# anacarsi/ss25_Hierarchical_Multiscale_Image_Classification

Measured on AMD Instinct MI355X. Metric: 224x224 patches/sec (ResNet18 fwd), higher is better.
Workload: dtype bf16; 1 GPU; resnet18_fwd_872k_patches_bf16; input=uint8 HWC patches resident in HBM, outputs=features[B,512] + logits[B,2] + labels, weights=seeded random init, parallelism=single GPU

## Files before the change

### ss25_hierarchical_multiscale_image_classification_amd/csrc/halo16.h

```cpp
#pragma once
#include "conv_device.h"

namespace hipac {

template <typename T> struct Elem16;
template <> struct Elem16<__bf16> {
  static __device__ __forceinline__ f32x4 mfma(bf16x8 a, bf16x8 b, f32x4 c) {
    return __builtin_amdgcn_mfma_f32_16x16x32_bf16(a, b, c, 0, 0, 0);
  }
};
template <> struct Elem16<_Float16> {
  static __device__ __forceinline__ f32x4 mfma(f16x8 a, f16x8 b, f32x4 c) {
    return __builtin_amdgcn_mfma_f32_16x16x32_f16(a, b, c, 0, 0, 0);
  }
};

template <typename T> struct Asm16;
template <> struct Asm16<__bf16> {
  static __device__ __forceinline__ void mfma(f32x4& c, const bf16x8& a, const bf16x8& b) {
    asm volatile("v_mfma_f32_16x16x32_bf16 %0, %1, %2, %0" : "+v"(c) : "v"(a), "v"(b));
  }
};
template <> struct Asm16<_Float16> {
  static __device__ __forceinline__ void mfma(f32x4& c, const f16x8& a, const f16x8& b) {
    asm volatile("v_mfma_f32_16x16x32_f16 %0, %1, %2, %0" : "+v"(c) : "v"(a), "v"(b));
  }
};
template <int OFF, typename F>
__device__ __forceinline__ void lds_read16(F& f, unsigned addr) {
  static_assert(OFF >= 0 && OFF < 65536, "ds offset field");
  asm volatile("ds_read_b128 %0, %1 offset:%2" : "=v"(f) : "v"(addr), "n"(OFF));
}
#if defined(__HIP_DEVICE_COMPILE__)
__device__ __forceinline__ void permlane16_swap(unsigned& a, unsigned& b) {
  const auto r = __builtin_amdgcn_permlane16_swap(a, b, false, false);
  a = r[0];
  b = r[1];
}
#else
__device__ inline void permlane16_swap(unsigned&, unsigned&) {}
#endif
template <int N>
__device__ __forceinline__ void wait_lgkmcnt() {
  static_assert(N >= 0 && N < 16, "lgkmcnt range");
  asm volatile("s_waitcnt lgkmcnt(%0)" ::"n"(N));
}

template <int STRIDE> __host__ __device__ constexpr int b16_tap(int k) { return STRIDE == 1 ? k : (int)((0x471538620ull >> (4 * k)) & 15); }
template <int STRIDE> __host__ __device__ constexpr int b16_kh(int k) { return b16_tap<STRIDE>(k) / 3; }
template <int STRIDE> __host__ __device__ constexpr int b16_kw(int k) { return b16_tap<STRIDE>(k) % 3; }
__host__ __device__ constexpr int perm16(int n) { return n < 4 ? 2 * n : (n < 12 ? 2 * n - 7 : 2 * n - 16); }
__host__ __device__ constexpr int perm16_inv(int j) { return (j & 1) ? (j + 7) / 2 : (j < 8 ? j / 2 : j / 2 + 8); }

#ifndef HIPAC_H16_EPI_PRIO
#define HIPAC_H16_EPI_PRIO 0
#endif
#ifndef HIPAC_H16_STAGE16
#define HIPAC_H16_STAGE16 0
#endif
#ifndef HIPAC_H16_ABL
#define HIPAC_H16_ABL 0
#endif
#ifndef HIPAC_H16_AHEAD
#define HIPAC_H16_AHEAD 3
#endif

constexpr int kPoolSlots = 7;

#if defined(__HIP_DEVICE_COMPILE__)
template <int CTRL>
__device__ __forceinline__ float dpp_add(float v) {
  return v + __builtin_bit_cast(float, __builtin_amdgcn_update_dpp(0, __builtin_bit_cast(int, v), CTRL, 0xf, 0xf, false));
}
__device__ __forceinline__ float row16_sum(float v) {
  v = dpp_add<0x128>(v);
  v = dpp_add<0x124>(v);
  v = dpp_add<0x122>(v);
  return dpp_add<0x121>(v);
}
#else
__device__ inline float row16_sum(float v) { return v; }
#endif

template <typename T, int CIN, int COUT, int H, int W, int BM, int BN, int NSW, bool RELU, bool RESID, bool OUTF32, int PCIN = 0,
          bool POOL = false, bool S2 = false>
__global__ __launch_bounds__(256, 2) void conv3x3_halo16_kernel(const T* __restrict__ in, const T* __restrict__ wgt,
                                                                const float* __restrict__ bias, const T* __restrict__ resid,
                                                                void* __restrict__ outp, int M, int n_img, int n_mtiles,
                                                                const char* __restrict__ zero_page,
                                                                const T* __restrict__ wgt_p = nullptr) {
  using E = Elem<T>;
  using frag = typename E::frag;
  constexpr int CC = CIN / 64;
  constexpr int KTOT = 9 * CIN;
  constexpr int WM = 2, WN = 2;
  constexpr int WPX = BM / WM;
  constexpr int MT = WPX / 16;
  constexpr int WTN = BN / WN, NT = WTN / 16;
  constexpr int A_PIECES = halo_band_pieces(W, BM);
  constexpr int A_BYTES = A_PIECES * 1024;
  constexpr int W_BYTES = BN * 128;
  constexpr int WPW = BN / 8 / 4;
  constexpr int NTILES_N = COUT / BN;
  constexpr int PCC = PCIN / 64;
  constexpr int NSTEP = 9 * CC + PCC;
  static_assert(sizeof(T) == 2, "16-bit operands");
  static_assert(!S2 || (PCIN == 0 && !RESID && !POOL && !OUTF32), "stride-2 form: plain entry conv");
  static_assert(!POOL || (OUTF32 && RELU && (BM + H * W - 1) / (H * W) + 1 <= kPoolSlots && H * W > 16),
                "pooled epilogue: the fp32 form of the direct epilogue, maps of more than 16 pixels");
  static_assert(PCIN % 64 == 0 && (PCIN == 0 || !RESID), "folded projection replaces the residual input");
  static_assert((BM == 128 || BM == 256) && WTN % 16 == 0 && COUT % BN == 0 && CIN % 64 == 0 && MT <= 8, "tile shape");
  static_assert((BN / 8) % 4 == 0, "W piece split");
  static_assert(NSW == 2 || NSW == 3, "weight ring depth");
  constexpr int SROWW = WTN * 4 + 16;
  constexpr int STG_BYTES = 4 * 32 * SROWW;
  constexpr int S_BYTES = NSW * W_BYTES > STG_BYTES ? NSW * W_BYTES : STG_BYTES;
  static_assert(A_BYTES + S_BYTES <= 80 * 1024, "LDS: two workgroups per CU");
  static_assert(BM + 2 * W + 4 <= A_PIECES * 8, "band slots");

  extern __shared__ __attribute__((aligned(1024))) unsigned char ring[];
  unsigned char* const Abuf = ring;
  unsigned char* const Wbuf = ring + A_BYTES;

  const int tid = threadIdx.x;
  const int lane = tid & 63;
  const int wave = __builtin_amdgcn_readfirstlane(tid >> 6);
  const int wm = wave % WM, wn = wave / WM;
  const int n16 = lane & 15, g = lane >> 4;
  const int pn = n16 < 4 ? 2 * n16 : (n16 < 12 ? 2 * n16 - 7 : 2 * n16 - 16);

  using gptr_t = const __attribute__((address_space(1))) void*;
  using lptr_t = __attribute__((address_space(3))) void*;
  const char* in_b = reinterpret_cast<const char*>(in);
  const char* w_b = reinterpret_cast<const char*>(wgt);
  const int prow = lane >> 3, dchunk = lane & 7;

  const rsrc_t a_rsrc = make_rsrc(in_b, S2 ? n_img * (4 * H * W * CIN * 2) : M * CIN * 2);
  const int a_lane = (prow * CIN + (dchunk ^ ((4 * wave + (prow >> 1)) & 7)) * 8) * 2;
  constexpr int NPB = S2 ? (A_PIECES + 3) / 4 : 1;
  int b_pix[NPB];
  auto plane_offsets = [&](int m0_) {
    if constexpr (S2) {
#pragma unroll
      for (int k = 0; k < NPB; ++k) {
        const int q = 8 * (wave + 4 * k) + prow;
        const int u = m0_ - W - 3 + q;
        const int b = u / (H * W), rem = u - b * (H * W), r = rem / W, c = rem - r * W;
        b_pix[k] = (q >= 2 && u >= 0 && u < M) ? (b * (2 * H) + 2 * r) * (2 * W) + 2 * c : -1;
      }
    }
  };
  auto issue_plane_band = [&](int k, int cc) {
    if constexpr (S2) {
      const int py = k < 4 ? 1 : (k < 6 ? 0 : (k < 8 ? 1 : 0)), px = k < 6 ? 1 : 0;
      const int pofs = (py * 2 * W + px) * CIN * 2 + cc * 128 + (dchunk ^ ((4 * wave + (prow >> 1)) & 7)) * 16;
#pragma unroll
      for (int kk = 0; kk < NPB; ++kk) {
        const int p = wave + 4 * kk;
        if (p < A_PIECES) buffer_load_lds16(a_rsrc, Abuf + p * 1024, b_pix[kk] < 0 ? (int)0x80000000 : b_pix[kk] * (CIN * 2) + pofs, 0);
      }
    }
  };
  auto issue_band_of = [&](int m0_, int cc) {
    const int mlast_ = (m0_ + BM <= M ? m0_ + BM : M) - 1;
    const int npieces_ = (mlast_ - m0_ + 1 + 2 * W + 2 + 2 + 7) >> 3;
    const int base = ((m0_ - W - 3) * CIN + cc * 64) * 2;
    for (int p = wave; p < npieces_; p += 4) {
      int off = a_lane + base + p * (8 * CIN * 2);
      if (p == 0 && prow < 2) off = (int)0x80000000;
      buffer_load_lds16(a_rsrc, Abuf + p * 1024, off, 0);
    }
  };

  constexpr int N_EPI_STORES = MT * (OUTF32 ? NT : NT / 2);
  bool prev_full = false;
  for (int vb = blockIdx.x, first_tile = 1;; vb += gridDim.x, first_tile = 0) {
  const int xcd = vb & 7, slot = vb >> 3;
  const int mt_q = (n_mtiles + 7) >> 3;
  const int mt = (slot / NTILES_N) < mt_q ? xcd * mt_q + slot / NTILES_N : n_mtiles;
  const int nt = slot % NTILES_N;
  if (mt >= n_mtiles) break;
  const int m0 = mt * BM, n0 = nt * BN;
  const int mlast = (m0 + BM <= M ? m0 + BM : M) - 1;
  const int mstart = m0 - W - 1;
  HALO_STAMP(t_start);
  int w_off[WPW];
  int wp_off[PCC > 0 ? WPW : 1];
#pragma unroll
  for (int i = 0; i < WPW; ++i) {
    const int row = (wave + 4 * i) * 8 + prow;
    const int j = row & 15;
    const int srow = (row & ~15) | ((j & 1) ? (j + 7) >> 1 : (j < 8 ? j >> 1 : (j >> 1) + 8));
    w_off[i] = ((n0 + srow) * KTOT + (dchunk ^ ((row >> 1) & 7)) * 8) * 2;
    if constexpr (PCC > 0) wp_off[i] = ((n0 + srow) * PCIN + (dchunk ^ ((row >> 1) & 7)) * 8) * 2;
  }
  const rsrc_t w_rsrc = make_rsrc(w_b, COUT * KTOT * 2);
  const rsrc_t wp_rsrc = make_rsrc(PCC > 0 ? reinterpret_cast<const char*>(wgt_p) : w_b, COUT * (PCC > 0 ? PCIN : KTOT) * 2);
  auto issue_w = [&](int step, int slot_) {
    if (PCC > 0 && step >= 9 * CC) {
      const int kofs_bytes = (step - 9 * CC) * 128;
      static_for<WPW>([&](auto I) {
        constexpr int i = decltype(I)::value;
        buffer_load_lds16(wp_rsrc, Wbuf + slot_ * W_BYTES + (wave + 4 * i) * 1024, wp_off[PCC > 0 ? i : 0], kofs_bytes);
      });
      asm volatile("" ::: "memory");
      return;
    }
    const int cc = step / 9, tap = step - cc * 9;
    const int kofs_bytes = ((S2 ? b16_tap<2>(tap) : tap) * CIN + cc * 64) * 2;
    static_for<WPW>([&](auto I) {
      constexpr int i = decltype(I)::value;
      buffer_load_lds16(w_rsrc, Wbuf + slot_ * W_BYTES + (wave + 4 * i) * 1024, w_off[i], kofs_bytes);
    });
  };
  auto issue_gather = [&](int pc) {
    if constexpr (PCC > 0) {
      const int npx_ = mlast - m0 + 1;
      const int first = W + 3, last = first + npx_ - 1;
      for (int p = wave + (first >> 3); p <= (last >> 3); p += 4) {
        const int q = p * 8 + prow;
        const int mm = m0 + q - first;
        const bool ok = q >= first && q <= last;
        const int b = mm / (H * W), rem = mm - b * (H * W), y = rem / W, x = rem - y * W;
        const int schunk = dchunk ^ ((q >> 1) & 7);
        const char* src = ok ? reinterpret_cast<const char*>(resid) +
                                   ((((size_t)b * (2 * H) + 2 * y) * (2 * W) + 2 * x) * PCIN + pc * 64 + schunk * 8) * 2
                             : zero_page + dchunk * 16;
        __builtin_amdgcn_global_load_lds((gptr_t)src, (lptr_t)(Abuf + p * 1024), 16, 0, 0);
      }
    }
  };

  const int mw0 = m0 + wm * WPX + pn;
  const int q0 = mw0 - mstart + 2;
  unsigned epk = 0;
  {
    const int rem = mw0 % (H * W);
    int y = rem / W, x = rem - y * W;
#pragma unroll
    for (int i = 0; i < MT; ++i) {
      epk |= (unsigned)((x == 0 ? 1 : 0) | (!S2 && x == W - 1 ? 2 : 0) | (y == 0 ? 4 : 0) | (!S2 && y == H - 1 ? 8 : 0)) << (4 * i);
      x += 16 % W, y += 16 / W;
      if (x >= W) x -= W, y += 1;
      if (y >= H) y -= H;
    }
  }
  HALO_STAMP(t_setup);
  const int ck0 = g << 4;
  const int rdw0 = (wn * WTN + pn) * 128 + ((g ^ ((pn >> 1) & 7)) << 4);

  f32x4 acc[MT][NT];
#pragma unroll
  for (int i = 0; i < MT; ++i)
#pragma unroll
    for (int j = 0; j < NT; ++j) acc[i][j] = f32x4{0.f, 0.f, 0.f, 0.f};

  const unsigned lds0 = (unsigned)(unsigned long long)(lptr_t)ring;
  auto k_step = [&](const unsigned char* wst, const int (&a_addr)[MT], auto&& mid) {
    constexpr int AH = HIPAC_H16_AHEAD;
    constexpr int NS = 2 * MT;
    static_assert(AH >= 1 && AH <= 3 && MT >= 2 + NT, "read-ahead schedule");
    frag wf[2][NT];
    frag af[AH + 1];
    const unsigned w0 = lds0 + (unsigned)(wst - ring) + (unsigned)rdw0;
    const unsigned w1 = w0 ^ 64u;
    unsigned aa[NS];
#pragma unroll
    for (int i = 0; i < MT; ++i) aa[i] = lds0 + (unsigned)a_addr[i], aa[MT + i] = aa[i] ^ 64u;
    static_for<NT>([&](auto J) { lds_read16<decltype(J)::value * 2048>(wf[0][decltype(J)::value], w0); });
    static_for<AH>([&](auto S) { lds_read16<0>(af[decltype(S)::value], aa[decltype(S)::value]); });
    __builtin_amdgcn_s_setprio(1);
    static_for<NS>([&](auto S) {
      constexpr int s = decltype(S)::value, kk = s / MT, i = s % MT;
      if constexpr (s + AH < NS) lds_read16<0>(af[(s + AH) % (AH + 1)], aa[s + AH]);
      if constexpr (s >= 1 && s <= NT) lds_read16<(s - 1) * 2048>(wf[1][s - 1], w1);
      constexpr int a_after = (s + AH < NS ? AH : NS - 1 - s);
      constexpr int w_lo = (s - AH > 1 ? s - AH : 1), w_hi = (s < NT ? s : NT);
      constexpr int w_after = w_hi >= w_lo ? w_hi - w_lo + 1 : 0;
      static_assert(MT - AH >= NT, "W1 fragments are older than the first activation fragment that needs them");
      if constexpr (!(HIPAC_H16_ABL & 4)) wait_lgkmcnt<a_after + w_after>();
#pragma unroll
      for (int j = 0; j < NT; ++j) Asm16<T>::mfma(acc[i][j], wf[kk][j], af[s % (AH + 1)]);
      if constexpr (s == MT / 2) mid();
    });
    __builtin_amdgcn_s_setprio(0);
  };

#ifdef HIPAC_HALO_STAMPS
  unsigned long long t_first = 0;
#endif
  int s = 0;
  if constexpr (S2) plane_offsets(m0);
  if (first_tile) {
    if constexpr (S2) issue_plane_band(0, 0);
    else issue_band_of(m0, 0);
  }
  if (first_tile) {
#pragma unroll
    for (int pstep = 0; pstep < NSW - 1; ++pstep)
      if (pstep < NSTEP) issue_w(pstep, pstep);
  }
  for (int cc = 0; cc < CC; ++cc) {
    if (cc > 0) {
      __builtin_amdgcn_s_barrier();
      if constexpr (S2) issue_plane_band(0, cc);
      else issue_band_of(m0, cc);
    }
#pragma unroll HIPAC_HALO_TAP_UNROLL
    for (int tap = 0; tap < 9; ++tap, ++s) {
      if (S2 && !(HIPAC_H16_ABL & 64) && (tap == 4 || tap == 6 || tap == 8)) {
        __builtin_amdgcn_s_barrier();
        issue_plane_band(tap, cc);
      }
      if (NSW == 3 && tap != 0 && s + 1 < NSTEP) wait_vmcnt<WPW>();
      else if (s == 0 && prev_full) wait_vmcnt<N_EPI_STORES>();
      else if (!(HIPAC_H16_ABL & 8) || tap == 0) wait_vmcnt<0>();
      if (!(HIPAC_H16_ABL & 1) || tap == 0) __builtin_amdgcn_s_barrier();
#ifdef HIPAC_HALO_STAMPS
      if (s == 0) {
        t_first = __builtin_amdgcn_s_memtime();
        __builtin_amdgcn_s_waitcnt(0xC07F);
      }
#endif
      const int tap_w = S2 ? b16_tap<2>(tap) : tap;
      const int kh = tap_w / 3, kw = tap_w - kh * 3;
      const int toff = S2 ? (kh == 0 ? -W : 0) + (kw == 0 ? -1 : 0) : (kh - 1) * W + kw - 1;
      const unsigned char* wst = Wbuf + (s % NSW) * W_BYTES;
      const unsigned tapmask = ((kw == 0 ? 1u : 0u) | (!S2 && kw == 2 ? 2u : 0u) | (kh == 0 ? 4u : 0u) | (!S2 && kh == 2 ? 8u : 0u)) * 0x11111111u;
      const int qt = q0 + toff;
      const int x0 = ck0 ^ (((qt >> 1) & 7) << 4);
      const int a_in = (qt << 7) + x0;
      const int a_zero = ((qt & 1) << 7) + x0;
      unsigned em;
      asm("v_and_b32 %0, %1, %2" : "=v"(em) : "s"(tapmask), "v"(epk));
// ... 222 lines not shown
```

### ss25_hierarchical_multiscale_image_classification_amd/csrc/stem.h

```cpp
#pragma once
#include <type_traits>
#include "conv_device.h"
#include "halo16x2.h"

namespace hipac {

constexpr int kStemTilesPerImage = 56;

template <typename T, bool U8IN>
__global__ __launch_bounds__(256, 2) void stem_pool_kernel(const void* __restrict__ xin_, const T* __restrict__ wgt,
                                                        const float* __restrict__ bias, T* __restrict__ out,
                                                        int n_tiles, const unsigned short* __restrict__ lut_t,
                                                        long long in_bytes) {
  const T* xin = reinterpret_cast<const T*>(xin_);
  using E = Elem<T>;
  using frag = typename E::frag;
  constexpr int PTH = 8, PTW = 7;
  constexpr int STW = 2 * PTW + 1, STH = 2 * PTH + 1, NPX = STW * STH;
  constexpr int PROWS = 2 * STH + 5, PCOLS = 36;
  static_assert(56 / PTW * (56 / PTH) == kStemTilesPerImage, "tile count");
  constexpr int PPR = PCOLS / 2;
  constexpr int NPIECE = PROWS * PPR;
  constexpr int PF = (NPIECE + 255) / 256;
  constexpr int TILES_X = 56 / PTW, TILES_Y = 56 / PTH, TPI = TILES_X * TILES_Y;
  constexpr int SPX = 144;
  constexpr int P_BYTES = PROWS * PCOLS * 8, S_BYTES = 256 * SPX;
  constexpr int RAWROW = (PCOLS * 3 + 3 + 3) / 4 * 4, RAWDW = RAWROW / 4;
  constexpr int RAW_BYTES = U8IN ? PROWS * RAWROW + 3 * 256 * 2 : 0;
  constexpr int NRAW = PROWS * RAWDW, PFR = (NRAW + 255) / 256;
  __shared__ __attribute__((aligned(16))) unsigned char smem[2 * P_BYTES + S_BYTES + RAW_BYTES];
  unsigned char* const Sl = smem + 2 * P_BYTES;
  unsigned char* const Rl = smem + 2 * P_BYTES + S_BYTES;
  unsigned short* const Ll = reinterpret_cast<unsigned short*>(Rl + PROWS * RAWROW);

  const int tid = threadIdx.x, lane = tid & 63, wave = tid >> 6;
  const int r = lane & 31, h = lane >> 5;

  if constexpr (U8IN) {
    for (int i = threadIdx.x; i < 3 * 256; i += 256) Ll[i] = lut_t[i];
  }
  frag wreg[2][7][2];
  {
    const char* wb = reinterpret_cast<const char*>(wgt) + r * 448 + 16 * h;
#pragma unroll
    for (int j = 0; j < 2; ++j)
#pragma unroll
      for (int kh = 0; kh < 7; ++kh)
#pragma unroll
        for (int kk = 0; kk < 2; ++kk)
          wreg[j][kh][kk] = *reinterpret_cast<const frag*>(wb + j * 32 * 448 + kh * 64 + kk * 32);
  }
  float4 bv[2][4];
#pragma unroll
  for (int j = 0; j < 2; ++j)
#pragma unroll
    for (int q = 0; q < 4; ++q) bv[j][q] = *reinterpret_cast<const float4*>(bias + j * 32 + 8 * q + 4 * h);

  int P[2], a_rd[2], ly[2], lx[2], sidx[2];
#pragma unroll
  for (int i = 0; i < 2; ++i) {
    P[i] = (2 * wave + i) * 32 + r;
    const int Pc = P[i] < NPX ? P[i] : NPX - 1;
    ly[i] = Pc / STW;
    lx[i] = Pc - ly[i] * STW;
    sidx[i] = P[i] < NPX ? ly[i] * STW + lx[i] : P[i];
    a_rd[i] = ((2 * ly[i]) * PCOLS + 2 * lx[i]) * 8 + 16 * h;
  }

  auto tile_origin = [&](int tile, int& b, int& py0, int& px0) {
    b = tile / TPI;
    const int t = tile - b * TPI;
    const int ty = t / TILES_X;
    py0 = ty * PTH;
    px0 = (t - ty * TILES_X) * PTW;
  };
  u32x4 pre[U8IN ? 1 : PF];
  unsigned praw[U8IN ? PFR : 1];
  auto fetch = [&](int tile) {
    int b, py0, px0;
    tile_origin(tile, b, py0, px0);
    const int R0 = 2 * (2 * py0 - 1), C0 = 2 * (2 * px0 - 1);
    if constexpr (U8IN) {
      const unsigned char* src = reinterpret_cast<const unsigned char*>(xin_);
      const int sh = ((C0 - 3) * 3) & 3;
      const long long tile_base = (((long long)b * kPatch + (R0 - 3)) * kPatch + (C0 - 3)) * 3 - sh;
      const long long lo = -tile_base, hi = in_bytes - 4 - tile_base;
      const int lo32 = lo > 0 ? (lo < 0x7fffffff ? (int)lo : 0x7fffffff) : 0;
      const int hi32 = hi < 0 ? -1 : (hi < 0x7fffffff ? (int)hi : 0x7fffffff);
      static_for<PFR>([&](auto I) {
        constexpr int k = decltype(I)::value;
        const int i = tid + 256 * k;
        const int row = i / RAWDW, j = i - row * RAWDW;
        const int y = R0 + row - 3;
        const int voff = row * (kPatch * 3) + 4 * j;
        const bool ok = i < NRAW && (unsigned)y < (unsigned)kPatch && voff >= lo32 && voff <= hi32;
        const unsigned v = *reinterpret_cast<const unsigned*>(src + tile_base + (ok ? voff : lo32));
        praw[k] = ok ? v : 0u;
      });
    } else {
      const char* img = reinterpret_cast<const char*>(xin) + (size_t)b * kPadH * kPadW * 8;
      static_for<PF>([&](auto I) {
        constexpr int k = decltype(I)::value;
        const int i = tid + 256 * k;
        const int row = i / PPR, cp = i - row * PPR;
        const int R = R0 + row, C = C0 + 2 * cp;
        const bool ok = i < NPIECE && R >= 0 && C >= 0 && R < kPadH && C + 1 < kPadW;
        const u32x4 v = *reinterpret_cast<const u32x4*>(img + (ok ? ((size_t)R * kPadW + C) * 8 : 0));
        pre[k] = ok ? v : u32x4{0u, 0u, 0u, 0u};
      });
    }
  };
  auto stash = [&](int buf) {
    if constexpr (U8IN) {
      static_for<PFR>([&](auto I) {
        constexpr int k = decltype(I)::value;
        const int i = tid + 256 * k;
        if (i < NRAW) *reinterpret_cast<unsigned*>(Rl + i * 4) = praw[k];
      });
    } else {
      static_for<PF>([&](auto I) {
        constexpr int k = decltype(I)::value;
        const int i = tid + 256 * k;
        if (i < NPIECE) *reinterpret_cast<u32x4*>(smem + buf * P_BYTES + i * 16) = pre[k];
      });
    }
  };
  auto convert = [&](int tile, int buf) {
    int b, py0, px0;
    tile_origin(tile, b, py0, px0);
    const int R0 = 2 * (2 * py0 - 1), C0 = 2 * (2 * px0 - 1);
    const int sh = ((C0 - 3) * 3) & 3;
    for (int i = tid; i < NPIECE; i += 256) {
      const int row = i / PPR, cp = i - row * PPR;
      const int y = R0 + row - 3;
      const unsigned char* rr = Rl + row * RAWROW + sh + 6 * cp;
      u32x4 v = {0u, 0u, 0u, 0u};
      if ((unsigned)y < (unsigned)kPatch) {
#pragma unroll
        for (int px = 0; px < 2; ++px) {
          const int x = C0 + 2 * cp + px - 3;
          if ((unsigned)x < (unsigned)kPatch) {
            const unsigned c0 = Ll[rr[3 * px + 0]], c1 = Ll[256 + rr[3 * px + 1]], c2 = Ll[512 + rr[3 * px + 2]];
            v[2 * px] = c0 | (c1 << 16);
            v[2 * px + 1] = c2;
          }
        }
      }
      *reinterpret_cast<u32x4*>(smem + buf * P_BYTES + i * 16) = v;
    }
  };

  int tile = blockIdx.x;
  if (tile < n_tiles) {
    fetch(tile);
    stash(0);
    if constexpr (U8IN) {
      __syncthreads();
      convert(tile, 0);
    }
  }
  __syncthreads();
  for (int it = 0; tile < n_tiles; tile += gridDim.x, ++it) {
    const int buf = it & 1;
    const bool more = tile + (int)gridDim.x < n_tiles;
    if (more) fetch(tile + gridDim.x);
    int b, py0, px0;
    tile_origin(tile, b, py0, px0);
    const int sy0 = 2 * py0 - 1, sx0 = 2 * px0 - 1;
    const unsigned char* Pl = smem + buf * P_BYTES;

    f32x16 acc[2][2];
#pragma unroll
    for (int i = 0; i < 2; ++i)
#pragma unroll
      for (int j = 0; j < 2; ++j)
#pragma unroll
        for (int e = 0; e < 16; ++e) acc[i][j][e] = 0.f;
#ifdef HIPAC_ABL_STEM_NO_MFMA
    if (n_tiles < 0)
#endif
#pragma unroll
    for (int kh = 0; kh < 7; ++kh) {
#pragma unroll
      for (int kk = 0; kk < 2; ++kk) {
        frag af[2];
#pragma unroll
        for (int i = 0; i < 2; ++i) af[i] = *reinterpret_cast<const frag*>(Pl + a_rd[i] + kh * (PCOLS * 8) + kk * 32);
#pragma unroll
        for (int i = 0; i < 2; ++i)
#pragma unroll
          for (int j = 0; j < 2; ++j) acc[i][j] = E::mfma(wreg[j][kh][kk], af[i], acc[i][j]);
      }
    }
#ifdef HIPAC_ABL_STEM_NO_EPI
    if (n_tiles < 0)
#endif
#pragma unroll
    for (int i = 0; i < 2; ++i) {
      const bool inside = (sy0 + ly[i]) >= 0 && (sx0 + lx[i]) >= 0 && P[i] < NPX;
      const unsigned inside_mask = inside ? 0xffffffffu : 0u;
#pragma unroll
      for (int j = 0; j < 2; ++j)
#pragma unroll
        for (int q = 0; q < 4; ++q) {
          typename E::vec4 ov;
          ov[0] = (T)fmaxf(acc[i][j][4 * q + 0] + bv[j][q].x, 0.f);
          ov[1] = (T)fmaxf(acc[i][j][4 * q + 1] + bv[j][q].y, 0.f);
          ov[2] = (T)fmaxf(acc[i][j][4 * q + 2] + bv[j][q].z, 0.f);
          ov[3] = (T)fmaxf(acc[i][j][4 * q + 3] + bv[j][q].w, 0.f);
          u32x2 pk = __builtin_bit_cast(u32x2, ov);
          pk[0] &= inside_mask;
          pk[1] &= inside_mask;
          *reinterpret_cast<u32x2*>(Sl + sidx[i] * SPX + (j * 32 + 8 * q + 4 * h) * 2) = pk;
        }
    }
    __syncthreads();
    if (more) stash(buf ^ 1);
#ifdef HIPAC_ABL_STEM_NO_POOL
    if (n_tiles < 0)
#endif
    for (int item = tid; item < PTH * PTW * 8; item += 256) {
      const int pp = item >> 3, c8 = item & 7;
      const int py = pp / PTW, px = pp - py * PTW;
      s16x8 best = {0, 0, 0, 0, 0, 0, 0, 0};
#pragma unroll
      for (int dy = 0; dy < 3; ++dy)
#pragma unroll
        for (int dx = 0; dx < 3; ++dx)
          best = __builtin_elementwise_max(
              best, *reinterpret_cast<const s16x8*>(Sl + ((2 * py + dy) * STW + 2 * px + dx) * SPX + c8 * 16));
      const frag o = __builtin_bit_cast(frag, best);
      *reinterpret_cast<frag*>(out + (((size_t)b * 56 + py0 + py) * 56 + px0 + px) * 64 + c8 * 8) = o;
    }
    __syncthreads();
    if constexpr (U8IN) {
#ifndef HIPAC_ABL_STEM_NO_CONVERT
      if (more) convert(tile + gridDim.x, buf ^ 1);
#endif
      __syncthreads();
    }
  }
}

#if defined(__HIP_DEVICE_COMPILE__)
__device__ __forceinline__ void buffer_load_lds4(rsrc_t rs, void* lds, int voffset, int soffset) {
  __builtin_amdgcn_raw_ptr_buffer_load_lds(rs, (__attribute__((address_space(3))) void*)lds, 4, voffset, soffset, 0, 0);
}
#else
__device__ inline void buffer_load_lds4(rsrc_t, void*, int, int) {}
#endif
constexpr int kStripSteps = 14;

#ifndef HIPAC_STRIP_PRIO
#define HIPAC_STRIP_PRIO 2
#endif
template <typename T, bool SPLIT = false, bool Q8 = false>
__global__ __launch_bounds__(512, 2) void stem_pool_strip2_kernel(const unsigned char* __restrict__ x,
                                                                  const T* __restrict__ wgt,
                                                                  const float* __restrict__ btab, T* __restrict__ out,
                                                                  int n_strips, int in_bytes, unsigned char* __restrict__ out_q = nullptr) {
  using E = Elem<T>;
  using frag = typename E::frag;
  static_assert(!SPLIT || std::is_same<T, _Float16>::value, "split pairs are fp16");
  static_assert(!Q8 || SPLIT, "the q8 tensor belongs to the pair layout");
  constexpr int OPIX = SPLIT ? 128 : 64;
  constexpr int WLO_BYTES = SPLIT ? 2 * 12 * 1024 : 0;
  constexpr int NRP = 11, PXW = 128;
  constexpr int PLANE = NRP * PXW * 4;
  constexpr int PATCH_BYTES = 3 * PLANE;
  constexpr int RAW_PITCH = 512, RAW_ROWS = 22;
  constexpr int RAW_BYTES = RAW_ROWS * RAW_PITCH;
  constexpr int TEAM_BYTES = PATCH_BYTES + RAW_BYTES;
  constexpr int CARRY_BYTES = 512 * 64;
  constexpr int STG_BYTES = 4 * 14 * 64;
  __shared__ __attribute__((aligned(16))) unsigned char smem[2 * TEAM_BYTES + CARRY_BYTES + 8 * STG_BYTES + 4096 + WLO_BYTES];

  const int tid = threadIdx.x, lane = tid & 63;
  const int wave = __builtin_amdgcn_readfirstlane(tid >> 6);
  const int team = wave >> 2, tw = wave & 3;
  const int jt = tw & 1, st = tw >> 1;
  const int r = lane & 31, h = lane >> 5;
  unsigned char* const Pl = smem + team * TEAM_BYTES;
  unsigned char* const Rl = Pl + PATCH_BYTES;
  unsigned char* const Cl = smem + 2 * TEAM_BYTES + tid * 16;
  unsigned char* const Sl = smem + 2 * TEAM_BYTES + CARRY_BYTES + wave * STG_BYTES;
  float* const Bl = reinterpret_cast<float*>(smem + 2 * TEAM_BYTES + CARRY_BYTES + 8 * STG_BYTES);
  for (int i = tid; i < 16 * 64; i += 512) Bl[i] = btab[i];
  int s_off[4];
#pragma unroll
  for (int m = 0; m < 4; ++m) {
    const int c = lane + 64 * m, pix = c >> 2;
    const int q = (pix * 147) >> 11, k = pix - 14 * q;
    s_off[m] = SPLIT ? ((q & 1) * 56 + k) * 128 + (q >> 1) * 64 + (c & 3) * 8 : (q * 56 + k) * 64 + (c & 3) * 8;
  }
  int q_off[2];
#pragma unroll
  for (int m = 0; m < 2; ++m) {
    const int c = lane + 64 * m, pix = c >> 2;
    const int q = pix >= 14 ? 1 : 0, k = pix - 14 * q;
    q_off[m] = (q * 56 + k) * 128 + (c & 3) * 8;
  }

  const float unscale = SPLIT ? btab[16 * 64] : 1.f;
  frag wreg[12];
  unsigned char* const Wl = smem + 2 * TEAM_BYTES + CARRY_BYTES + 8 * STG_BYTES + 4096 + jt * (12 * 1024) + lane * 16;
  {
    const char* wb = reinterpret_cast<const char*>(wgt) + (size_t)(jt * 32 + r) * (192 * 2) + 16 * h;
    if constexpr (SPLIT) {
      if (team == 0 && st == 0) {
#pragma unroll
        for (int s = 0; s < 12; ++s)
          *reinterpret_cast<frag*>(Wl + s * 1024) = *reinterpret_cast<const frag*>(wb + 64 * 192 * 2 + s * 32);
      }
    }
#pragma unroll
    for (int s = 0; s < 12; ++s) wreg[s] = *reinterpret_cast<const frag*>(wb + s * 32);
#pragma unroll
    for (int s = 0; s < 12; ++s) asm volatile("" ::"v"(wreg[s]));
  }
  const rsrc_t in_rsrc = make_rsrc(x, in_bytes);

  auto issue_dma = [&](int strip, int ys) {
    const int b = strip >> 1, side = strip & 1;
    const int base = b * (kPatch * kPatch * 3) + (16 * ys - 3) * (kPatch * 3) + 3 * (112 * side - 5) - 1;
    const int sub = lane >> 5, ch16 = lane & 31;
    const bool col_ok = ch16 < 25 && (side == 0 ? ch16 >= 1 : ch16 < 22);
    static_for<3>([&](auto K) {
      constexpr int k = decltype(K)::value;
      if (tw < 3 || k < 2) {
        const int row = 6 * tw + 2 * k + sub;
        const int iy = 16 * ys - 3 + row;
        const bool ok = col_ok && (unsigned)iy < (unsigned)kPatch && row < 21;
        buffer_load_lds16(in_rsrc, Rl + (6 * tw + 2 * k) * RAW_PITCH, ok ? base + row * (kPatch * 3) + ch16 * 16 : (int)0x80000000, 0);
      }
    });
  };

  const int cRp = 3 * tw + (lane >> 4), cxg = lane & 15;
  const bool ctask = (lane >> 4) < (tw < 3 ? 3 : 2);
  const unsigned char* const craw = Rl + (2 * cRp) * RAW_PITCH + cxg * 24;
  unsigned char* const cdst = Pl + cRp * (PXW * 4) + cxg * 32;
  auto convert = [&](int strip, int ys) {
    (void)strip, (void)ys;
    if (!ctask) return;
    unsigned da[7], db[7];
    {
      const u32x2 a0 = *reinterpret_cast<const u32x2*>(craw), a1 = *reinterpret_cast<const u32x2*>(craw + 8),
                  a2 = *reinterpret_cast<const u32x2*>(craw + 16);
      const u32x2 b0 = *reinterpret_cast<const u32x2*>(craw + RAW_PITCH),
                  b1 = *reinterpret_cast<const u32x2*>(craw + RAW_PITCH + 8),
                  b2 = *reinterpret_cast<const u32x2*>(craw + RAW_PITCH + 16);
      da[0] = a0[0], da[1] = a0[1], da[2] = a1[0], da[3] = a1[1], da[4] = a2[0], da[5] = a2[1];
      db[0] = b0[0], db[1] = b0[1], db[2] = b1[0], db[3] = b1[1], db[4] = b2[0], db[5] = b2[1];
      da[6] = *reinterpret_cast<const unsigned*>(craw + 24);
      db[6] = *reinterpret_cast<const unsigned*>(craw + RAW_PITCH + 24);
    }
#pragma unroll
    for (int c = 0; c < 3; ++c) {
      unsigned o[8];
#pragma unroll
      for (int px = 0; px < 8; ++px) {
        const int w = 1 + 3 * px + c;
        o[px] = PackPair<T>::pack((float)((da[w >> 2] >> (8 * (w & 3))) & 0xffu) - 128.f,
                                  (float)((db[w >> 2] >> (8 * (w & 3))) & 0xffu) - 128.f);
      }
      *reinterpret_cast<u32x4*>(cdst + c * PLANE) = u32x4{o[0], o[1], o[2], o[3]};
      *reinterpret_cast<u32x4*>(cdst + c * PLANE + 16) = u32x4{o[4], o[5], o[6], o[7]};
    }
  };

  const unsigned char* const fbase = Pl + (2 * r + 56 * st) * 4 + 16 * h;
  const int tg = 2 * blockIdx.x + team, tstride = 2 * gridDim.x;
  const int my_strips = tg < n_strips ? (n_strips - tg + tstride - 1) / tstride : 0;
  const int n_steps = my_strips * kStripSteps;
  const int max_strips = (n_strips - 2 * (int)blockIdx.x + tstride - 1) / tstride;
  const int n_phases = 2 * max_strips * kStripSteps + 2;

#ifdef HIPAC_HALO_STAMPS
  unsigned long long z_sum[6] = {0, 0, 0, 0, 0, 0};
#endif
  f32x16 acc[8];
  const bool first_col_wave = st == 0;
  for (int p = 0; p < n_phases; ++p) {
    const int hs = p - team - 1;
    HALO_STAMP(z_t0);
    if (hs >= -1 && hs < 2 * n_steps) {
      const int n = hs >> 1;
      if (hs & 1) {
#if HIPAC_STRIP_PRIO == 2
        __builtin_amdgcn_s_setprio(1);
#endif
        const int strip = tg + ((n < 0 ? 0 : n) / kStripSteps) * tstride;
        const int ys = (n < 0 ? 0 : n) % kStripSteps;
#ifdef HIPAC_ABL_STRIP_NO_EPI
#pragma unroll
        for (int i = 0; i < 8; ++i) asm volatile("" ::"v"(acc[i]));
        if (n_strips < 0)
#endif
        if (n >= 0) {
          const int b = strip >> 1, side = strip & 1;
          f32x16 carry;
#pragma unroll
          for (int k = 0; k < 4; ++k) {
            const f32x4 cv = *reinterpret_cast<const f32x4*>(Cl + k * 8192);
#pragma unroll
            for (int t = 0; t < 4; ++t) carry[4 * k + t] = ys == 0 ? -3.0e38f : cv[t];
          }
          const bool writer = (r & 1) == 0 && r <= 26;
          const bool col_m1 = side == 0 && first_col_wave && r == 0;
#ifdef HIPAC_ABL_STRIP_STORE_LOCAL
          T* const dst0 = out + (size_t)blockIdx.x * 16384 + jt * 32 + (b & 0);
#else
          T* const dst0 = out + ((((size_t)b * 56 + 4 * ys) * 56 + 28 * side + 14 * st) * OPIX + jt * 32);
#endif
          typedef __attribute__((ext_vector_type(2))) short s16x2;
          auto flush_pair = [&](int g) {
            asm volatile("s_waitcnt lgkmcnt(0)" ::: "memory");
#pragma unroll
            for (int m = 0; m < 4; ++m)
              if (m < 3 || lane < 32)
                store16_out(dst0 + g * (2 * 56 * 128) + s_off[m], *reinterpret_cast<const u32x4*>(Sl + (lane + 64 * m) * 16));
            if constexpr (Q8) {
              unsigned char* const qdst0 = out_q + ((((size_t)b * 56 + 4 * ys) * 56 + 28 * side + 14 * st) * 128 + jt * 32) + g * (2 * 56 * 128);
#pragma unroll
              for (int m = 0; m < 2; ++m)
                if (m < 1 || lane < 48) {
                  const f16x8 hv = *reinterpret_cast<const f16x8*>(Sl + (lane + 64 * m) * 16);
                  const f16x8 lv = *reinterpret_cast<const f16x8*>(Sl + (lane + 64 * m + 112) * 16);
                  u32x2 h8, l8;
#pragma unroll
                  for (int k = 0; k < 2; ++k) {
                    h8[k] = cvt4_e4m3((float)hv[4 * k], (float)hv[4 * k + 1], (float)hv[4 * k + 2], (float)hv[4 * k + 3]);
                    l8[k] = cvt4_e4m3((float)lv[4 * k] * kQ8LoScale, (float)lv[4 * k + 1] * kQ8LoScale, (float)lv[4 * k + 2] * kQ8LoScale,
                                      (float)lv[4 * k + 3] * kQ8LoScale);
                  }
                  *reinterpret_cast<u32x2*>(qdst0 + q_off[m]) = l8;
                  *reinterpret_cast<u32x2*>(qdst0 + q_off[m] + 64) = h8;
                }
            }
            asm volatile("s_waitcnt lgkmcnt(0)" ::: "memory");
          };
          static_for<4>([&](auto Q) {
            constexpr int q = decltype(Q)::value;
            unsigned pk[8];
            unsigned lk_prev = 0;
            (void)lk_prev;
            if constexpr (SPLIT) {
#pragma unroll
              for (int d = 0; d < 8; ++d) {
                float pv[2];
#pragma unroll
                for (int t = 0; t < 2; ++t) {
                  const int e = 2 * d + t;
                  const float top = q == 0 ? carry[e] : acc[q == 0 ? 0 : 2 * q - 1][e];
                  const float a0 = col_m1 ? -3.0e38f : fmaxf(fmaxf(top, acc[2 * q][e]), acc[2 * q + 1][e]);
                  const float a1 = __builtin_bit_cast(float, __builtin_amdgcn_update_dpp(0, __builtin_bit_cast(int, a0), 0x130, 0xf, 0xf, false));
                  const float t1 = fmaxf(a0, a1);
                  const float u2 = __builtin_bit_cast(float, __builtin_amdgcn_update_dpp(0, __builtin_bit_cast(int, t1), 0x130, 0xf, 0xf, false));
                  pv[t] = fmaxf(fmaxf(t1, u2), 0.f) * unscale;
                }
                const f16x2 h2 = __builtin_convertvector(f32x2{pv[0], pv[1]}, f16x2);
                const f16x2 l2 = __builtin_convertvector(f32x2{pv[0] - (float)h2[0], pv[1] - (float)h2[1]}, f16x2);
                pk[d] = __builtin_bit_cast(unsigned, h2);
                if (writer && (d & 1))
                  *reinterpret_cast<u32x2*>(Sl + ((2 + (q & 1)) * 14 + (r >> 1)) * 64 + (d >> 1) * 16 + h * 8) =
                      u32x2{lk_prev, __builtin_bit_cast(unsigned, l2)};
                lk_prev = __builtin_bit_cast(unsigned, l2);
              }
            } else {
#pragma unroll
            for (int cq = 0; cq < 4; ++cq) {
              float v[4];
#pragma unroll
              for (int t = 0; t < 4; ++t) {
                const int e = 4 * cq + t;
                const float top = q == 0 ? carry[e] : acc[q == 0 ? 0 : 2 * q - 1][e];
                v[t] = fmaxf(fmaxf(top, acc[2 * q][e]), acc[2 * q + 1][e]);
              }
              pk[2 * cq] = PackPair<T>::pack_rn(v[0], v[1]);
              pk[2 * cq + 1] = PackPair<T>::pack_rn(v[2], v[3]);
            }
            }
            if constexpr (!SPLIT)
#pragma unroll
            for (int d = 0; d < 8; ++d) {
              const unsigned a0 = col_m1 ? 0x80008000u : pk[d];
              const unsigned a1 = __builtin_amdgcn_update_dpp(0u, a0, 0x130, 0xf, 0xf, false);
              const s16x2 t1 = __builtin_elementwise_max(__builtin_bit_cast(s16x2, a0), __builtin_bit_cast(s16x2, a1));
              const unsigned u2 = __builtin_amdgcn_update_dpp(0u, __builtin_bit_cast(unsigned, t1), 0x130, 0xf, 0xf, false);
              const s16x2 t2 = __builtin_elementwise_max(t1, __builtin_bit_cast(s16x2, u2));
              pk[d] = __builtin_bit_cast(unsigned, __builtin_elementwise_max(t2, s16x2{0, 0}));
            }
            if (writer) {
#pragma unroll
              for (int cq = 0; cq < 4; ++cq)
                *reinterpret_cast<u32x2*>(Sl + ((SPLIT ? (q & 1) : q) * 14 + (r >> 1)) * 64 + cq * 16 + h * 8) = u32x2{pk[2 * cq], pk[2 * cq + 1]};
            }
            if constexpr (SPLIT && q == 1) flush_pair(0);
          });
#pragma unroll
          for (int k = 0; k < 4; ++k)
            *reinterpret_cast<f32x4*>(Cl + k * 8192) = f32x4{acc[7][4 * k], acc[7][4 * k + 1], acc[7][4 * k + 2], acc[7][4 * k + 3]};
          if constexpr (SPLIT) {
            flush_pair(1);
          } else {
          asm volatile("s_waitcnt lgkmcnt(0)" ::: "memory");
#ifdef HIPAC_ABL_STRIP_NO_STORE
          if (n_strips < 0)
#endif
#pragma unroll
          for (int m = 0; m < 4; ++m)
            if (m < 3 || lane < 32)
              store16_out(dst0 + s_off[m], *reinterpret_cast<const u32x4*>(Sl + (lane + 64 * m) * 16));
          }
        }
        HALO_STAMP(z_te);
#ifdef HIPAC_HALO_STAMPS
        if (n >= 0) z_sum[1] += z_te - z_t0, z_sum[4] += 1;
#endif
        if (n + 1 < n_steps) {
          const int gn = n + 1;
          if (n < 0) {
            issue_dma(tg, 0);
            wait_vmcnt<0>();
          } else {
            wait_vmcnt<Q8 ? 16 : SPLIT ? 8 : 4>();
          }
          HALO_STAMP(z_tw);
#ifdef HIPAC_ABL_STRIP_NO_CONVERT
          if (n_strips < 0)
#endif
          convert(tg + (gn / kStripSteps) * tstride, gn % kStripSteps);
#ifdef HIPAC_HALO_STAMPS
          asm volatile("s_waitcnt lgkmcnt(0)" ::: "memory");
          HALO_STAMP(z_tc);
          if (n >= 0) z_sum[2] += z_tw - z_te, z_sum[3] += z_tc - z_tw;
#endif
          asm volatile("s_waitcnt lgkmcnt(0)" ::: "memory");
#ifdef HIPAC_ABL_STRIP_NO_DMA
          if (n_strips < 0)
#endif
          if (gn + 1 < n_steps) issue_dma(tg + ((gn + 1) / kStripSteps) * tstride, (gn + 1) % kStripSteps);
        }
      } else {
        f32x16 binit;
        {
          const int strip1 = tg + (n / kStripSteps) * tstride, ys1 = n % kStripSteps, side1 = strip1 & 1;
          const int cc = (side1 == 0 && st == 0) ? (r == 1 ? 1 : (r == 2 ? 2 : 0)) : ((side1 == 1 && st == 1 && r == 28) ? 3 : 0);
          const float* bl = Bl + cc * 64 + jt * 32 + 4 * h;
#pragma unroll
          for (int q = 0; q < 4; ++q) {
            const float4 v = *reinterpret_cast<const float4*>(bl + 8 * q);
            binit[4 * q + 0] = v.x, binit[4 * q + 1] = v.y, binit[4 * q + 2] = v.z, binit[4 * q + 3] = v.w;
          }
          acc[0] = binit, acc[1] = binit, acc[7] = binit;
          if (ys1 == 0 || ys1 == kStripSteps - 1) {
            static_for<3>([&](auto RC) {
              constexpr int rc = decltype(RC)::value + 1;
              constexpr int i = rc == 1 ? 0 : (rc == 2 ? 1 : 7);
              if ((rc == 3) == (ys1 != 0)) {
#pragma unroll
                for (int q = 0; q < 4; ++q) {
                  const float4 v = *reinterpret_cast<const float4*>(bl + rc * 256 + 8 * q);
                  acc[i][4 * q + 0] = v.x, acc[i][4 * q + 1] = v.y, acc[i][4 * q + 2] = v.z, acc[i][4 * q + 3] = v.w;
                }
              }
            });
          }
        }
#if HIPAC_STRIP_PRIO == 1
        __builtin_amdgcn_s_setprio(1);
#endif
#ifdef HIPAC_ABL_STRIP_NO_MFMA
        if (n_strips < 0)
#endif
        {
          frag ring3[3];
          auto rd = [&](auto F) {
            constexpr int f = decltype(F)::value;
            const unsigned char* pp = fbase + f * (PXW * 4);
            const u32x2 lo = *reinterpret_cast<const u32x2*>(pp), hi = *reinterpret_cast<const u32x2*>(pp + 8);
            ring3[f % 3] = __builtin_bit_cast(frag, u32x4{lo[0], lo[1], hi[0], hi[1]});
          };
          frag wlo[SPLIT ? 4 : 1];
          auto rdw = [&](int c_) {
            if constexpr (SPLIT) {
#pragma unroll
              for (int rp = 0; rp < 4; ++rp) wlo[rp] = *reinterpret_cast<const frag*>(Wl + (c_ * 4 + rp) * 1024);
            }
          };
          rdw(0);
          rd(std::integral_constant<int, 0>{});
          rd(std::integral_constant<int, 1>{});
          static_for<33>([&](auto F) {
            constexpr int f = decltype(F)::value, c = f / NRP, j = f % NRP;
            if constexpr (f + 2 < 33) rd(std::integral_constant<int, f + 2>{});
            static_for<4>([&](auto RP) {
              constexpr int rp = decltype(RP)::value, i = j - rp;
              if constexpr (i >= 0 && i < 8) {
                if constexpr (c == 0 && rp == 0 && i >= 2 && i <= 6) acc[i] = E::mfma(wreg[0], ring3[f % 3], binit);
                else acc[i] = E::mfma(wreg[c * 4 + rp], ring3[f % 3], acc[i]);
              }
            });
            if constexpr (SPLIT) {
              static_for<4>([&](auto RP) {
                constexpr int rp = decltype(RP)::value, i = j - rp;
                if constexpr (i >= 0 && i < 8) acc[i] = E::mfma(wlo[rp], ring3[f % 3], acc[i]);
              });
              if constexpr (j == NRP - 1 && c < 2) rdw(c + 1);
            }
            __builtin_amdgcn_sched_barrier(0);
          });
        }
#if HIPAC_STRIP_PRIO == 1
        __builtin_amdgcn_s_setprio(0);
#endif
#ifdef HIPAC_HALO_STAMPS
#pragma unroll
        for (int i = 0; i < 8; ++i) asm volatile("" ::"v"(acc[i]));
        HALO_STAMP(z_tm);
        z_sum[0] += z_tm - z_t0;
#endif
      }
    }
    HALO_STAMP(z_tb0);
#if HIPAC_STRIP_PRIO == 2
    __builtin_amdgcn_s_setprio(0);
#endif
    asm volatile("s_waitcnt lgkmcnt(0)" ::: "memory");
    __builtin_amdgcn_s_barrier();
#ifdef HIPAC_HALO_STAMPS
    HALO_STAMP(z_tb1);
    z_sum[5] += z_tb1 - z_tb0;
#endif
  }
#ifdef HIPAC_HALO_STAMPS
  if (lane == 0) {
    atomicAdd(&g_halo_stamps[0], z_sum[0]);
    atomicAdd(&g_halo_stamps[1], z_sum[1]);
    atomicAdd(&g_halo_stamps[2], z_sum[2]);
    atomicAdd(&g_halo_stamps[4], z_sum[3]);
    atomicAdd(&g_halo_stamps[5], z_sum[5]);
    atomicAdd(&g_halo_stamps[3], z_sum[4]);
  }
#endif
}

}
```

Baseline: 307,000 patches/s.

## Hand-schedule stem strip MFMA loop with inline asm, deeper LDS prefetch, swizzled staging

Replaces the compiler-scheduled MFMA loop in the stem strip kernel with inline-asm 32x32x16 MFMAs, explicit ds_read_b64 prefetches running 2-4 fragments ahead, and compile-time-computed lgkmcnt waits. The sched barriers go away, and weight reads for the split path are spread across the loop. The epilogue staging buffer gets an XOR-swizzled layout to cut LDS bank conflicts, and DPP moves switch to bound_ctrl mov_dpp. The priority macro is hardcoded to the default mode. Hand-counted waitcnts and s_nop padding risk hazards or stalls if the counts are wrong.

```diff
diff --git a/ss25_hierarchical_multiscale_image_classification_amd/csrc/halo16.h b/ss25_hierarchical_multiscale_image_classification_amd/csrc/halo16.h
--- a/ss25_hierarchical_multiscale_image_classification_amd/csrc/halo16.h
+++ b/ss25_hierarchical_multiscale_image_classification_amd/csrc/halo16.h
@@ -24,12 +24,34 @@
 template <> struct Asm16<_Float16> {
   static __device__ __forceinline__ void mfma(f32x4& c, const f16x8& a, const f16x8& b) {
     asm volatile("v_mfma_f32_16x16x32_f16 %0, %1, %2, %0" : "+v"(c) : "v"(a), "v"(b));
+  }
+};
+template <typename T> struct Asm32;
+template <> struct Asm32<__bf16> {
+  static __device__ __forceinline__ void mfma(f32x16& c, const bf16x8& a, const bf16x8& b) {
+    asm volatile("v_mfma_f32_32x32x16_bf16 %0, %1, %2, %0" : "+v"(c) : "v"(a), "v"(b));
+  }
+  static __device__ __forceinline__ void mfma_init(f32x16& d, const bf16x8& a, const bf16x8& b, const f32x16& c) {
+    asm volatile("v_mfma_f32_32x32x16_bf16 %0, %1, %2, %3" : "=&v"(d) : "v"(a), "v"(b), "v"(c));
+  }
+};
+template <> struct Asm32<_Float16> {
+  static __device__ __forceinline__ void mfma(f32x16& c, const f16x8& a, const f16x8& b) {
+    asm volatile("v_mfma_f32_32x32x16_f16 %0, %1, %2, %0" : "+v"(c) : "v"(a), "v"(b));
+  }
+  static __device__ __forceinline__ void mfma_init(f32x16& d, const f16x8& a, const f16x8& b, const f32x16& c) {
+    asm volatile("v_mfma_f32_32x32x16_f16 %0, %1, %2, %3" : "=&v"(d) : "v"(a), "v"(b), "v"(c));
   }
 };
 template <int OFF, typename F>
 __device__ __forceinline__ void lds_read16(F& f, unsigned addr) {
   static_assert(OFF >= 0 && OFF < 65536, "ds offset field");
   asm volatile("ds_read_b128 %0, %1 offset:%2" : "=v"(f) : "v"(addr), "n"(OFF));
+}
+template <int OFF, typename F>
+__device__ __forceinline__ void lds_read8(F& f, unsigned addr) {
+  static_assert(OFF >= 0 && OFF < 65536, "ds offset field");
+  asm volatile("ds_read_b64 %0, %1 offset:%2" : "=v"(f) : "v"(addr), "n"(OFF));
 }
 #if defined(__HIP_DEVICE_COMPILE__)
 __device__ __forceinline__ void permlane16_swap(unsigned& a, unsigned& b) {
diff --git a/ss25_hierarchical_multiscale_image_classification_amd/csrc/stem.h b/ss25_hierarchical_multiscale_image_classification_amd/csrc/stem.h
--- a/ss25_hierarchical_multiscale_image_classification_amd/csrc/stem.h
+++ b/ss25_hierarchical_multiscale_image_classification_amd/csrc/stem.h
@@ -251,9 +251,28 @@
 #endif
 constexpr int kStripSteps = 14;
 
-#ifndef HIPAC_STRIP_PRIO
-#define HIPAC_STRIP_PRIO 2
-#endif
+template <bool SPLIT> constexpr int kStripAhead = SPLIT ? 2 : 4;
+constexpr int kStripFrags = 33;
+template <bool SPLIT, int AH>
+constexpr int strip_wait(int f) {
+  int n = 0, frag_done[kStripFrags + AH] = {}, w_done[3][4] = {};
+  if (SPLIT)
+    for (int rp = 0; rp < 4; ++rp) w_done[0][rp] = ++n;
+  for (int g = 0; g < AH; ++g) frag_done[g] = (n += 2);
+  for (int g = 0; g < kStripFrags; ++g) {
+    const int c = g / 11, j = g % 11;
+    if (g + AH < kStripFrags) frag_done[g + AH] = (n += 2);
+    if (g == f) {
+      int need = frag_done[g];
+      if (SPLIT)
+        for (int rp = 0; rp < 4; ++rp)
+          if (j - rp >= 0 && j - rp < 8 && w_done[c][rp] > need) need = w_done[c][rp];
+      return n - need;
+    }
+    if (SPLIT && j >= 7 && c < 2) w_done[c + 1][j - 7] = ++n;
+  }
+  return 0;
+}
 template <typename T, bool SPLIT = false, bool Q8 = false>
 __global__ __launch_bounds__(512, 2) void stem_pool_strip2_kernel(const unsigned char* __restrict__ x,
                                                                   const T* __restrict__ wgt,
@@ -369,7 +388,10 @@
     }
   };
 
-  const unsigned char* const fbase = Pl + (2 * r + 56 * st) * 4 + 16 * h;
+  const unsigned lds_base = (unsigned)(size_t)(__attribute__((address_space(3))) unsigned char*)smem;
+  const unsigned fb = lds_base + team * TEAM_BYTES + (2 * r + 56 * st) * 4 + 16 * h;
+  const unsigned wlb = lds_base + (unsigned)(Wl - smem);
+  (void)wlb;
   const int tg = 2 * blockIdx.x + team, tstride = 2 * gridDim.x;
   const int my_strips = tg < n_strips ? (n_strips - tg + tstride - 1) / tstride : 0;
   const int n_steps = my_strips * kStripSteps;
@@ -387,9 +409,7 @@
     if (hs >= -1 && hs < 2 * n_steps) {
       const int n = hs >> 1;
       if (hs & 1) {
-#if HIPAC_STRIP_PRIO == 2
         __builtin_amdgcn_s_setprio(1);
-#endif
         const int strip = tg + ((n < 0 ? 0 : n) / kStripSteps) * tstride;
         const int ys = (n < 0 ? 0 : n) % kStripSteps;
 #ifdef HIPAC_ABL_STRIP_NO_EPI
@@ -414,19 +434,27 @@
           T* const dst0 = out + ((((size_t)b * 56 + 4 * ys) * 56 + 28 * side + 14 * st) * OPIX + jt * 32);
 #endif
           typedef __attribute__((ext_vector_type(2))) short s16x2;
+          int kx = r >> 1, lx = lane;
+          asm volatile("" : "+v"(kx), "+v"(lx));
+          unsigned char* swz[4];
+#pragma unroll
+          for (int x = 0; x < 4; ++x) swz[x] = Sl + kx * 64 + ((x ^ (kx & 3)) * 16) + h * 8;
+          const unsigned char* const srd = Sl + (lx ^ ((lx >> 2) & 3)) * 16;
+          auto stg_wr = [&](int row, int cq) { return swz[cq ^ (2 * (row & 1))] + row * (14 * 64); };
+          auto stg_rd = [&](int o) { return srd + o * 16; };
           auto flush_pair = [&](int g) {
             asm volatile("s_waitcnt lgkmcnt(0)" ::: "memory");
 #pragma unroll
             for (int m = 0; m < 4; ++m)
               if (m < 3 || lane < 32)
-                store16_out(dst0 + g * (2 * 56 * 128) + s_off[m], *reinterpret_cast<const u32x4*>(Sl + (lane + 64 * m) * 16));
+                store16_out(dst0 + g * (2 * 56 * 128) + s_off[m], *reinterpret_cast<const u32x4*>(stg_rd(64 * m)));
             if constexpr (Q8) {
               unsigned char* const qdst0 = out_q + ((((size_t)b * 56 + 4 * ys) * 56 + 28 * side + 14 * st) * 128 + jt * 32) + g * (2 * 56 * 128);
 #pragma unroll
               for (int m = 0; m < 2; ++m)
                 if (m < 1 || lane < 48) {
-                  const f16x8 hv = *reinterpret_cast<const f16x8*>(Sl + (lane + 64 * m) * 16);
-                  const f16x8 lv = *reinterpret_cast<const f16x8*>(Sl + (lane + 64 * m + 112) * 16);
+                  const f16x8 hv = *reinterpret_cast<const f16x8*>(stg_rd(64 * m));
+                  const f16x8 lv = *reinterpret_cast<const f16x8*>(stg_rd(64 * m + 112));
                   u32x2 h8, l8;
 #pragma unroll
                   for (int k = 0; k < 2; ++k) {
@@ -441,7 +469,7 @@
             asm volatile("s_waitcnt lgkmcnt(0)" ::: "memory");
           };
           static_for<4>([&](auto Q) {
-            constexpr int q = decltype(Q)::value;
+            constexpr int q = decltype(Q)::value ^ 1;
             unsigned pk[8];
             unsigned lk_prev = 0;
             (void)lk_prev;
@@ -454,16 +482,16 @@
                   const int e = 2 * d + t;
                   const float top = q == 0 ? carry[e] : acc[q == 0 ? 0 : 2 * q - 1][e];
                   const float a0 = col_m1 ? -3.0e38f : fmaxf(fmaxf(top, acc[2 * q][e]), acc[2 * q + 1][e]);
-                  const float a1 = __builtin_bit_cast(float, __builtin_amdgcn_update_dpp(0, __builtin_bit_cast(int, a0), 0x130, 0xf, 0xf, false));
+                  const float a1 = __builtin_bit_cast(float, __builtin_amdgcn_mov_dpp(__builtin_bit_cast(int, a0), 0x130, 0xf, 0xf, true));
                   const float t1 = fmaxf(a0, a1);
-                  const float u2 = __builtin_bit_cast(float, __builtin_amdgcn_update_dpp(0, __builtin_bit_cast(int, t1), 0x130, 0xf, 0xf, false));
+                  const float u2 = __builtin_bit_cast(float, __builtin_amdgcn_mov_dpp(__builtin_bit_cast(int, t1), 0x130, 0xf, 0xf, true));
                   pv[t] = fmaxf(fmaxf(t1, u2), 0.f) * unscale;
                 }
                 const f16x2 h2 = __builtin_convertvector(f32x2{pv[0], pv[1]}, f16x2);
                 const f16x2 l2 = __builtin_convertvector(f32x2{pv[0] - (float)h2[0], pv[1] - (float)h2[1]}, f16x2);
                 pk[d] = __builtin_bit_cast(unsigned, h2);
                 if (writer && (d & 1))
-                  *reinterpret_cast<u32x2*>(Sl + ((2 + (q & 1)) * 14 + (r >> 1)) * 64 + (d >> 1) * 16 + h * 8) =
+                  *reinterpret_cast<u32x2*>(stg_wr(2 + (q & 1), d >> 1)) =
                       u32x2{lk_prev, __builtin_bit_cast(unsigned, l2)};
                 lk_prev = __builtin_bit_cast(unsigned, l2);
               }
@@ -485,18 +513,18 @@
 #pragma unroll
             for (int d = 0; d < 8; ++d) {
               const unsigned a0 = col_m1 ? 0x80008000u : pk[d];
-              const unsigned a1 = __builtin_amdgcn_update_dpp(0u, a0, 0x130, 0xf, 0xf, false);
+              const unsigned a1 = __builtin_amdgcn_mov_dpp(a0, 0x130, 0xf, 0xf, true);
               const s16x2 t1 = __builtin_elementwise_max(__builtin_bit_cast(s16x2, a0), __builtin_bit_cast(s16x2, a1));
-              const unsigned u2 = __builtin_amdgcn_update_dpp(0u, __builtin_bit_cast(unsigned, t1), 0x130, 0xf, 0xf, false);
+              const unsigned u2 = __builtin_amdgcn_mov_dpp(__builtin_bit_cast(unsigned, t1), 0x130, 0xf, 0xf, true);
               const s16x2 t2 = __builtin_elementwise_max(t1, __builtin_bit_cast(s16x2, u2));
               pk[d] = __builtin_bit_cast(unsigned, __builtin_elementwise_max(t2, s16x2{0, 0}));
             }
             if (writer) {
 #pragma unroll
               for (int cq = 0; cq < 4; ++cq)
-                *reinterpret_cast<u32x2*>(Sl + ((SPLIT ? (q & 1) : q) * 14 + (r >> 1)) * 64 + cq * 16 + h * 8) = u32x2{pk[2 * cq], pk[2 * cq + 1]};
+                *reinterpret_cast<u32x2*>(stg_wr(SPLIT ? (q & 1) : q, cq)) = u32x2{pk[2 * cq], pk[2 * cq + 1]};
             }
-            if constexpr (SPLIT && q == 1) flush_pair(0);
+            if constexpr (SPLIT && q == 0) flush_pair(0);
           });
 #pragma unroll
           for (int k = 0; k < 4; ++k)
@@ -511,7 +539,7 @@
 #pragma unroll
           for (int m = 0; m < 4; ++m)
             if (m < 3 || lane < 32)
-              store16_out(dst0 + s_off[m], *reinterpret_cast<const u32x4*>(Sl + (lane + 64 * m) * 16));
+              store16_out(dst0 + s_off[m], *reinterpret_cast<const u32x4*>(stg_rd(64 * m)));
           }
         }
         HALO_STAMP(z_te);
@@ -543,6 +571,19 @@
           if (gn + 1 < n_steps) issue_dma(tg + ((gn + 1) / kStripSteps) * tstride, (gn + 1) % kStripSteps);
         }
       } else {
+        constexpr int AH = kStripAhead<SPLIT>;
+        u32x2 ring[AH + 1][2];
+        auto rd = [&](auto F) {
+          constexpr int f = decltype(F)::value;
+          lds_read8<f * (PXW * 4)>(ring[f % (AH + 1)][0], fb);
+          lds_read8<f * (PXW * 4) + 8>(ring[f % (AH + 1)][1], fb);
+        };
+        frag wlo[SPLIT ? 4 : 1];
+        auto rdw = [&](auto C, auto RP) {
+          if constexpr (SPLIT) lds_read16<(decltype(C)::value * 4 + decltype(RP)::value) * 1024>(wlo[decltype(RP)::value], wlb);
+        };
+        static_for<4>([&](auto RP) { rdw(std::integral_constant<int, 0>{}, RP); });
+        static_for<AH>(rd);
         f32x16 binit;
         {
           const int strip1 = tg + (n / kStripSteps) * tstride, ys1 = n % kStripSteps, side1 = strip1 & 1;
@@ -568,53 +609,35 @@
             });
           }
         }
-#if HIPAC_STRIP_PRIO == 1
-        __builtin_amdgcn_s_setprio(1);
-#endif
 #ifdef HIPAC_ABL_STRIP_NO_MFMA
         if (n_strips < 0)
 #endif
         {
-          frag ring3[3];
-          auto rd = [&](auto F) {
-            constexpr int f = decltype(F)::value;
-            const unsigned char* pp = fbase + f * (PXW * 4);
-            const u32x2 lo = *reinterpret_cast<const u32x2*>(pp), hi = *reinterpret_cast<const u32x2*>(pp + 8);
-            ring3[f % 3] = __builtin_bit_cast(frag, u32x4{lo[0], lo[1], hi[0], hi[1]});
-          };
-          frag wlo[SPLIT ? 4 : 1];
-          auto rdw = [&](int c_) {
-            if constexpr (SPLIT) {
-#pragma unroll
-              for (int rp = 0; rp < 4; ++rp) wlo[rp] = *reinterpret_cast<const frag*>(Wl + (c_ * 4 + rp) * 1024);
-            }
-          };
-          rdw(0);
-          rd(std::integral_constant<int, 0>{});
-          rd(std::integral_constant<int, 1>{});
-          static_for<33>([&](auto F) {
+          using A32 = Asm32<T>;
+          asm volatile("" : "+v"(acc[0]), "+v"(acc[1]), "+v"(acc[7]), "+v"(binit));
+          static_for<kStripFrags>([&](auto F) {
             constexpr int f = decltype(F)::value, c = f / NRP, j = f % NRP;
-            if constexpr (f + 2 < 33) rd(std::integral_constant<int, f + 2>{});
+            if constexpr (f + AH < kStripFrags) rd(std::integral_constant<int, f + AH>{});
+            wait_lgkmcnt<strip_wait<SPLIT, AH>(f)>();
+            const u32x2 lo = ring[f % (AH + 1)][0], hi = ring[f % (AH + 1)][1];
+            const frag b = __builtin_bit_cast(frag, u32x4{lo[0], lo[1], hi[0], hi[1]});
             static_for<4>([&](auto RP) {
               constexpr int rp = decltype(RP)::value, i = j - rp;
               if constexpr (i >= 0 && i < 8) {
-                if constexpr (c == 0 && rp == 0 && i >= 2 && i <= 6) acc[i] = E::mfma(wreg[0], ring3[f % 3], binit);
-                else acc[i] = E::mfma(wreg[c * 4 + rp], ring3[f % 3], acc[i]);
+                if constexpr (c == 0 && rp == 0 && i >= 2 && i <= 6) A32::mfma_init(acc[i], wreg[0], b, binit);
+                else A32::mfma(acc[i], wreg[c * 4 + rp], b);
               }
             });
             if constexpr (SPLIT) {
               static_for<4>([&](auto RP) {
                 constexpr int rp = decltype(RP)::value, i = j - rp;
-                if constexpr (i >= 0 && i < 8) acc[i] = E::mfma(wlo[rp], ring3[f % 3], acc[i]);
+                if constexpr (i >= 0 && i < 8) A32::mfma(acc[i], wlo[rp], b);
               });
-              if constexpr (j == NRP - 1 && c < 2) rdw(c + 1);
+              if constexpr (j >= 7 && c < 2) rdw(std::integral_constant<int, c + 1>{}, std::integral_constant<int, j - 7>{});
             }
-            __builtin_amdgcn_sched_barrier(0);
           });
+          asm volatile("s_nop 7\n\ts_nop 7\n\ts_nop 3" ::: "memory");
         }
-#if HIPAC_STRIP_PRIO == 1
-        __builtin_amdgcn_s_setprio(0);
-#endif
 #ifdef HIPAC_HALO_STAMPS
 #pragma unroll
         for (int i = 0; i < 8; ++i) asm volatile("" ::"v"(acc[i]));
@@ -624,9 +647,7 @@
       }
     }
     HALO_STAMP(z_tb0);
-#if HIPAC_STRIP_PRIO == 2
     __builtin_amdgcn_s_setprio(0);
-#endif
     asm volatile("s_waitcnt lgkmcnt(0)" ::: "memory");
     __builtin_amdgcn_s_barrier();
 #ifdef HIPAC_HALO_STAMPS
```

Result: no change. 308,000 patches/s (median of 6 runs) (+0.3%).
